# EfficientMoE/MoE-Infinity

Measured on AMD Instinct MI355X. Metric: decode tokens/s through all MoE layers (expert-offload hot path), Mixtral-8x7B, device_memory_ratio=0.75, higher is better.
Workload: dtype bf16

## Files before the change

moe-infinity_amd/csrc/kernels.hip:

```cpp
#include "kdev.h"

#include <algorithm>

#include <type_traits>

#include <string.h>

namespace moeinf {

template <typename T>
__global__ __launch_bounds__(256) void retile_kernel(const T* __restrict__ src, char* __restrict__ dst, int R, int K) {
  constexpr int EPV = DT<T>::EPV;
  constexpr int EPT = 4 * EPV;
  const int KB = (K + EPT - 1) / EPT;
  const int lane = threadIdx.x & 63;
  const int kb = blockIdx.x * 4 + (threadIdx.x >> 6);
  const int rg = blockIdx.y;
  if (kb >= KB) return;
  const int row = rg * 16 + (lane & 15);
  const int k = kb * EPT + (lane >> 4) * EPV;
  u32x4 v = {0u, 0u, 0u, 0u};
  if (row < R && k < K) v = ld16(src + (size_t)row * K + k);
  *reinterpret_cast<u32x4*>(dst + ((size_t)rg * KB + kb) * 1024 + lane * 16) = v;
}
template <typename T>
__global__ __launch_bounds__(256) void retile_blob_kernel(RetileBlob b) {
  constexpr int EPV = DT<T>::EPV;
  constexpr int EPT = 4 * EPV;
  const int t = blockIdx.z;
  const char* src = reinterpret_cast<const char*>(b.src) + b.src_off[t];
  char* dst = reinterpret_cast<char*>(b.dst) + b.dst_off[t];
  const int R = b.R[t], K = b.K[t];
  if (K == 0) {
    const int64_t i = ((int64_t)blockIdx.y * gridDim.x + blockIdx.x) * 256 + threadIdx.x;
    if (i < R) reinterpret_cast<u32x4*>(dst)[i] = reinterpret_cast<const u32x4*>(src)[i];
    return;
  }
  const int KB = (K + EPT - 1) / EPT;
  const int lane = threadIdx.x & 63;
  const int kb = blockIdx.x * 4 + (threadIdx.x >> 6);
  const int rg = blockIdx.y;
  if (kb >= KB || rg * 16 >= R) return;
  const int row = rg * 16 + (lane & 15);
  const int k = kb * EPT + (lane >> 4) * EPV;
  u32x4 v = {0u, 0u, 0u, 0u};
  if (row < R && k < K) v = ld16(reinterpret_cast<const T*>(src) + (size_t)row * K + k);
  *reinterpret_cast<u32x4*>(dst + ((size_t)rg * KB + kb) * 1024 + lane * 16) = v;
}
hipError_t launch_retile_blob(const RetileBlob& b, int dtype, hipStream_t st) {
  const int ept = dtype == DT_F32 ? 16 : 32;
  unsigned gx = 1, gy = 1;
  for (int t = 0; t < b.n; ++t) {
    if (b.K[t] > 0) { gx = std::max(gx, (unsigned)(((b.K[t] + ept - 1) / ept + 3) / 4)); gy = std::max(gy, (unsigned)((b.R[t] + 15) / 16)); }
  }
  for (int t = 0; t < b.n; ++t)
    if (b.K[t] == 0) {
      const int64_t blocks = ((int64_t)b.R[t] + 255) / 256;
      while ((int64_t)gx * gy < blocks) gy += 1;
    }
  const dim3 grid(gx, gy, b.n);
  if (dtype != DT_F32) hipLaunchKernelGGL(retile_blob_kernel<uint16_t>, grid, dim3(256), 0, st, b);
  else hipLaunchKernelGGL(retile_blob_kernel<float>, grid, dim3(256), 0, st, b);
  return hipGetLastError();
}
template <typename T, bool F8>
__global__ __launch_bounds__(256) void pull_retile_kernel(RetileBlob b, unsigned long long* ts, int first) {
  if (ts && first && blockIdx.x == 0 && threadIdx.x == 0) ts[0] = (unsigned long long)wall_clock64();
  constexpr int EPV = DT<T>::EPV;
  constexpr int EPT = 4 * EPV;
  constexpr int W = F8 ? 2 : 1;
  constexpr int CK = 64 * EPV * W;
  constexpr int LROW = 1024 * W + 16;
  __shared__ __attribute__((aligned(16))) char lds[16 * LROW];
  __shared__ uint16_t lut[F8 ? 256 : 1];
  if (F8) {
    const uint32_t v8 = threadIdx.x, sg = v8 >> 7, ex = (v8 >> 3) & 15, m = v8 & 7;
    float f = (ex == 15 && m == 7) ? __builtin_nanf("") : (ex == 0 ? ldexpf((float)m, -9) : ldexpf(1.0f + (float)m * 0.125f, (int)ex - 7));
    if (sg) f = -f;
    lut[v8 & (F8 ? 255 : 0)] = (uint16_t)(__float_as_uint(f) >> 16);
    __syncthreads();
  }
  auto widen = [&](const u32x4 q, u32x4 (&o)[W]) {
    if constexpr (F8) {
      const uint32_t qq[4] = {q.x, q.y, q.z, q.w};
#pragma unroll
      for (int w = 0; w < 2; ++w) {
        uint32_t r4[4];
#pragma unroll
        for (int h2 = 0; h2 < 4; ++h2) {
          const uint32_t ww = qq[w * 2 + (h2 >> 1)], sh = (h2 & 1) * 16;
          r4[h2] = (uint32_t)lut[(ww >> sh) & 255] | ((uint32_t)lut[(ww >> (sh + 8)) & 255] << 16);
        }
        o[w] = u32x4{r4[0], r4[1], r4[2], r4[3]};
      }
    } else {
      o[0] = q;
    }
  };
  const int lane = threadIdx.x & 63, wave = threadIdx.x >> 6;
  int nunit[4], kcs[4], total = 0;
#pragma unroll
  for (int t = 0; t < 4; ++t) {
    kcs[t] = (t < b.n && b.K[t] > 0) ? (b.K[t] + CK - 1) / CK : 1;
    nunit[t] = t < b.n ? (b.K[t] > 0 ? ((b.R[t] + 15) / 16) * kcs[t] : (b.R[t] + 1024 * W - 1) / (1024 * W)) : 0;
    total += nunit[t];
  }
  u32x4 raw[4];
  uint32_t okmask = 0;
  constexpr int SRC_EPL = F8 ? 16 : EPV;
  auto decode = [&](int i, int& t, int& rg, int& kc) {
    t = 0;
    while (t < 3 && i >= nunit[t]) { i -= nunit[t]; ++t; }
    rg = i / kcs[t]; kc = i - rg * kcs[t];
  };
  auto load = [&](int i) {
    int t, rg, kc;
    decode(i, t, rg, kc);
    const char* src = reinterpret_cast<const char*>(b.src) + b.src_off[t];
    constexpr int SRC_ES = F8 ? 1 : (int)sizeof(T);
    okmask = 0;
#pragma unroll
    for (int j = 0; j < 4; ++j) {
      size_t elem;
      bool ok;
      if (b.K[t] > 0) {
        const int row = rg * 16 + wave * 4 + j, k = kc * CK + lane * SRC_EPL;
        ok = row < b.R[t] && k < b.K[t];
        elem = (size_t)min(row, b.R[t] - 1) * b.K[t] + min(k, b.K[t] - SRC_EPL);
      } else {
        const int piece = (rg * 1024 + (wave * 4 + j) * 64 + lane) * W;
        ok = piece < b.R[t];
        elem = (size_t)min(piece, b.R[t] - W) * EPV;
      }
      raw[j] = __builtin_nontemporal_load(reinterpret_cast<const u32x4*>(src + elem * SRC_ES));
      okmask |= (ok ? 1u : 0u) << j;
    }
  };
  int i = blockIdx.x;
  if (i < total) load(i);
  for (; i < total; i += gridDim.x) {
    int t, rg, kc;
    decode(i, t, rg, kc);
#pragma unroll
    for (int j = 0; j < 4; ++j) {
      u32x4 o[W];
      widen(raw[j], o);
#pragma unroll
      for (int w = 0; w < W; ++w) {
        if (!((okmask >> j) & 1u)) o[w] = u32x4{0u, 0u, 0u, 0u};
        *reinterpret_cast<u32x4*>(lds + (wave * 4 + j) * LROW + (lane * W + w) * 16) = o[w];
      }
    }
    __syncthreads();
// ... 348 lines not shown
}
__global__ __launch_bounds__(IDX_THREADS) void index_scatter_kernel(IndexArgs a, const int32_t* __restrict__ chunk_base) {
  const int npairs = a.T * a.K, E = a.E;
  const int p = blockIdx.x * IDX_THREADS + threadIdx.x;
  if (p < npairs) {
    const int rk = a.pair_slot[p];
    if (rk >= 0) {
      const int slot = chunk_base[(size_t)blockIdx.x * E + IDX_AT(a, p)] + rk;
      a.pair_slot[p] = slot;
      a.slot_token[slot] = p / a.K;
      a.slot_pair[slot] = p;
    }
  }
  if (a.shared) {
    const int base = a.offsets[E];
    for (int t = p; t < a.T; t += gridDim.x * IDX_THREADS) {
      a.slot_token[base + t] = t;
      a.slot_pair[base + t] = -1;
    }
  }
}
hipError_t launch_dispatch_index_wide(const IndexArgs& a, int32_t* chunk_scratch, hipStream_t st) {
  const int nchunks = (a.T * a.K + IDX_THREADS - 1) / IDX_THREADS;
  hipLaunchKernelGGL(index_count_kernel, dim3(nchunks), dim3(IDX_THREADS), 0, st, a, chunk_scratch);
  hipLaunchKernelGGL(index_scan_kernel, dim3(1), dim3(IDX_THREADS), 0, st, a, chunk_scratch, nchunks);
  hipLaunchKernelGGL(index_scatter_kernel, dim3(nchunks), dim3(IDX_THREADS), 0, st, a, chunk_scratch);
  return hipGetLastError();
}

hipError_t launch_dispatch_index(const IndexArgs& a, hipStream_t st) {
  hipLaunchKernelGGL(dispatch_index_kernel, dim3(1), dim3(IDX_THREADS), 0, st, a);
  return hipGetLastError();
}

__global__ __launch_bounds__(IDX_THREADS) void route_index_kernel(RouteArgs r, IndexArgs a, EpFuse pk) {
  __shared__ int wave_cnt[IDX_WAVES * IDX_MAXE];
  __shared__ int running[IDX_MAXE];
  __shared__ int offs[IDX_MAXE + 1];
  __shared__ int scan_tmp[IDX_MAXE];
  for (int t = threadIdx.x >> 6; t < r.T; t += IDX_WAVES) route_token(r, t, threadIdx.x & 63);
  __threadfence_block();
  __syncthreads();
  if (a.T * a.K <= 64 && !(a.capacity > 0 && a.T > a.rows)) {
    if (threadIdx.x < 64) index_small(a, running, offs);
  } else {
    index_body(a, wave_cnt, running, offs, scan_tmp);
  }
  if (pk.on) {
    __threadfence_block();
    __syncthreads();
    ep_pack_block_dt(pk, a.T * a.K, scan_tmp);
  }
}

template <typename T, int NW, int U>
__global__ __launch_bounds__(NW * 64) void route_shared2_kernel(RouteArgs r, IndexArgs a, FfnStage s, EpFuse pk) {
  __shared__ int running[IDX_MAXE];
  __shared__ int offs[IDX_MAXE + 1];
  __shared__ float red[NW][1][256];
  if (blockIdx.x == 0) {
    for (int t = threadIdx.x >> 6; t < r.T; t += NW) route_token(r, t, threadIdx.x & 63);
    __threadfence_block();
    __syncthreads();
    if (threadIdx.x < 64) index_small(a, running, offs);
    if (pk.on) {
      __syncthreads();
      ep_pack_block_dt(pk, a.T * a.K, reinterpret_cast<int*>(&red[0][0][0]));
    }
  } else {
    const char* W = reinterpret_cast<const char*>(s.wptr[s.E]);
    ffn_rows_item<T, 1, NW, U, 1>(s, (int)blockIdx.x - 1, W, true, r.T, 0, red);
  }
}
static EpFuse no_pack() {
  EpFuse f;
  memset(&f, 0, sizeof f);
  return f;
}
hipError_t launch_route_shared2(const RouteArgs& r, const IndexArgs& a, const FfnStage& s, hipStream_t st, const EpFuse* pack) {
  static const int nw = env_int("MOEINF_SH2_NW", 8), u = env_int("MOEINF_SH2_U", 4);
  const dim3 grid(1 + (s.R_sh + 15) / 16);
  const EpFuse pk = pack ? *pack : no_pack();
#define RS2(NWV, UU) hipLaunchKernelGGL((route_shared2_kernel<uint16_t, NWV, UU>), grid, dim3(NWV * 64), 0, st, r, a, s, pk)
  if (s.dtype == DT_F16) hipLaunchKernelGGL((route_shared2_kernel<half_t, 8, 4>), grid, dim3(512), 0, st, r, a, s, pk);
  else if (nw == 16) { if (u == 8) RS2(16, 8); else RS2(16, 4); }
  else if (nw == 4) { if (u == 8) RS2(4, 8); else RS2(4, 4); }
  else { if (u == 8) RS2(8, 8); else RS2(8, 4); }
#undef RS2
  return hipGetLastError();
}

template <typename T, int NMAT, int NW, int U>
__global__ __launch_bounds__(NW * 64) __attribute__((amdgpu_num_sgpr(80))) void ffn1_selfroute_kernel(RouteArgs r, IndexArgs a, FfnStage s, FfnStage sh2, int n_rg, int n_sh2) {
  using A = typename act_of<T>::type;
  __shared__ float red[NW][NMAT][256];
  __shared__ unsigned long long sh_w;
  __shared__ int sh_rank_ok;
  static_assert(sizeof(float) * NW * NMAT * 256 >= sizeof(int) * (2 * IDX_MAXE + 1), "index scratch aliases the reduction buffer");
  const int lane = threadIdx.x & 63;
  const int K = r.K, E = r.E;
  int b = (int)blockIdx.x - 1;
  if (n_sh2 < 0) {
    n_sh2 = -n_sh2;
    if (b >= 0) { const int n_routed = (int)gridDim.x - 1 - n_sh2; b = b < n_routed ? b + n_sh2 : b - n_routed; }
  }
  if (b >= 0 && b < n_sh2) {
    const char* Wsh = reinterpret_cast<const char*>(sh2.wptr[sh2.E]);
    ffn_rows_item<A, 1, NW, U, 1>(sh2, b, Wsh, true, 1, 0, reinterpret_cast<float (*)[1][256]>(&red[0][0][0]));
    return;
  }
  b -= n_sh2;
  if (b < 0) {
    if (threadIdx.x < 64) {
      int* scratch = reinterpret_cast<int*>(&red[0][0][0]);
      Routed o;
      route_core(r, 0, lane, o);
      int my_sel, rank;
      float my_w;
      route_store(r, 0, lane, o, &my_sel, &my_w, &rank);
      if (lane < K && s.dec_w) {
        s.dec_w[rank] = my_sel >= 0 ? s.wptr[my_sel] : 0ull;
        s.dec_cw[rank] = my_w;
      }
      __threadfence_block();
      index_small(a, scratch, scratch + IDX_MAXE);
    }
    return;
  }
  const int u = b / n_rg, rg = b - u * n_rg;
  if (threadIdx.x < 64) {
    uint64_t wp = 0;
    if (lane < E) wp = s.wptr[lane];
    uint64_t chosen = route_set_lean(r.logits, E, K, lane, r.kind == 2  ? r.x_dtype : DT_F32);
    for (int i = 0; i < u; ++i) chosen &= chosen - 1;
    const int e = chosen ? (int)__builtin_ctzll(chosen) : -1;
    uint64_t wsel = 0;
    if (e >= 0) {
      const uint32_t lo = (uint32_t)__builtin_amdgcn_readlane((int)(uint32_t)wp, e);
      const uint32_t hi = (uint32_t)__builtin_amdgcn_readlane((int)(uint32_t)(wp >> 32), e);
      wsel = ((uint64_t)hi << 32) | lo;
    }
    if (lane == 0) { sh_w = wsel; sh_rank_ok = e >= 0; }
  }
  __syncthreads();
  if (!sh_rank_ok) return;
  const char* W = reinterpret_cast<const char*>(sh_w);
  if (W == nullptr) {
    if (threadIdx.x == 0 && rg == 0) atomicExch(s.miss_flag, 1);
    return;
  }
  ffn_rows_item<A, NMAT, NW, U, 1, false, false, T>(s, rg, W, false, 1, u, red, 0);
}

static thread_local hipEvent_t t_timer_start = nullptr, t_timer_stop = nullptr;
void arm_kernel_timer(hipEvent_t start, hipEvent_t stop) { t_timer_start = start; t_timer_stop = stop; }
bool take_kernel_timer(hipEvent_t* start, hipEvent_t* stop) {
  if (!t_timer_stop) return false;
  *start = t_timer_start; *stop = t_timer_stop;
  t_timer_start = t_timer_stop = nullptr;
  return true;
}
hipError_t launch_ffn1_selfroute(const RouteArgs& r, const IndexArgs& a, const FfnStage& s1, const FfnStage* sh2, hipStream_t st) {
  const int n_rg = (s1.R + 15) / 16;
  const int n_sh2 = sh2 ? (sh2->R_sh + 15) / 16 : 0;
  const dim3 grid(n_sh2 + r.K * n_rg + 1);
  static const int lds_env = env_int("MOEINF_SR_LDS_KB", -1);
  const size_t dyn = (size_t)(lds_env >= 0 ? lds_env : (grid.x > 4 * 256 ? 30 : 0)) * 1024;
  static const int sr_u_env = env_int("MOEINF_SR_U", 0);
  const int sr_u = sr_u_env ? sr_u_env : (grid.x > 4 * 256 ? 4 : 8);
  if (s1.wdtype == DT_F8) {
    if (s1.epi != EPI_GATED_SILU || s1.dtype != DT_BF16) return hipErrorInvalidValue;
    if (sr_u == 8) KL((ffn1_selfroute_kernel<f8w_t, 2, 4, 8>), grid, dim3(256), dyn, st, r, a, s1, sh2 ? *sh2 : s1, n_rg, n_sh2);
    else KL((ffn1_selfroute_kernel<f8w_t, 2, 4, 4>), grid, dim3(256), dyn, st, r, a, s1, sh2 ? *sh2 : s1, n_rg, n_sh2);
    return hipGetLastError();
  }
  if (s1.epi != EPI_GATED_SILU) {
    if (s1.dtype == DT_BF16) KL((ffn1_selfroute_kernel<uint16_t, 1, 16, 4>), grid, dim3(1024), 0, st, r, a, s1, s1, n_rg, 0);
    else if (s1.dtype == DT_F16) KL((ffn1_selfroute_kernel<half_t, 1, 16, 4>), grid, dim3(1024), 0, st, r, a, s1, s1, n_rg, 0);
    else KL((ffn1_selfroute_kernel<float, 1, 16, 4>), grid, dim3(1024), 0, st, r, a, s1, s1, n_rg, 0);
    return hipGetLastError();
  }
  if (s1.dtype == DT_F16) {
    if (sr_u == 8) KL((ffn1_selfroute_kernel<half_t, 2, 4, 8>), grid, dim3(256), dyn, st, r, a, s1, sh2 ? *sh2 : s1, n_rg, n_sh2);
    else KL((ffn1_selfroute_kernel<half_t, 2, 4, 4>), grid, dim3(256), dyn, st, r, a, s1, sh2 ? *sh2 : s1, n_rg, n_sh2);
    return hipGetLastError();
  }
  static const int sr_order = env_int("MOEINF_SR_ORDER", 0);
  const int n_sh2_arg = (sr_order && n_sh2 > 0) ? -n_sh2 : n_sh2;
  if (sr_u == 8) KL((ffn1_selfroute_kernel<uint16_t, 2, 4, 8>), grid, dim3(256), dyn, st, r, a, s1, sh2 ? *sh2 : s1, n_rg, n_sh2_arg);
  else KL((ffn1_selfroute_kernel<uint16_t, 2, 4, 4>), grid, dim3(256), dyn, st, r, a, s1, sh2 ? *sh2 : s1, n_rg, n_sh2_arg);
  return hipGetLastError();
}

constexpr int SR_MAX_T = 8;
template <typename T, int NW, int U>
__global__ __launch_bounds__(NW * 64) __attribute__((amdgpu_num_sgpr(96))) void ffn1_selfroute_multi_kernel(RouteArgs r, IndexArgs a, FfnStage s, FfnStage sh2, int n_rg, int n_sh2) {
  using A = typename act_of<T>::type;
  __shared__ float red[NW][2][256];
  __shared__ int s_in[SR_MAX_T];
  __shared__ unsigned long long s_w;
  __shared__ int s_cnt, s_off;
  static_assert(sizeof(float) * NW * 2 * 256 >= sizeof(int) * (2 * IDX_MAXE + 1), "index scratch aliases the reduction buffer");
  const int lane = threadIdx.x & 63;
  const int Tn = r.T;
  int blk = (int)blockIdx.x - 1;
  if (blk < 0) {
    for (int t = threadIdx.x >> 6; t < Tn; t += NW) route_token(r, t, lane);
    __threadfence_block();
    __syncthreads();
    if (threadIdx.x < 64) {
      int* scratch = reinterpret_cast<int*>(&red[0][0][0]);
      index_small(a, scratch, scratch + IDX_MAXE);
    }
    return;
  }
  if (blk < n_sh2) {
    const char* Wsh = reinterpret_cast<const char*>(sh2.wptr[sh2.E]);
    ffn_rows_item<A, 1, NW, U, 1>(sh2, blk, Wsh, true, Tn, 0, reinterpret_cast<float (*)[1][256]>(&red[0][0][0]));
    return;
  }
  blk -= n_sh2;
  const int u = blk / n_rg, rg = blk - u * n_rg;
  if (threadIdx.x < 64) {
    uint64_t wp = 0;
    if (lane < r.E) wp = s.wptr[lane];
    uint64_t chosen[SR_MAX_T];
    uint64_t present = 0;
#pragma unroll
    for (int t = 0; t < SR_MAX_T; ++t) {
      chosen[t] = 0;
      if (t < Tn) chosen[t] = route_set_lean(r.logits + (size_t)t * r.E, r.E, r.K, lane);
      present |= chosen[t];
    }
    uint64_t m = present;
    for (int i = 0; i < u; ++i) m &= m - 1;
    const int e = m ? (int)__builtin_ctzll(m) : -1;
    int cnt = 0, off = 0;
    if (e >= 0) {
      const uint64_t below = (1ull << e) - 1ull;
#pragma unroll
      for (int t = 0; t < SR_MAX_T; ++t) {
        off += __popcll(chosen[t] & below);
        if ((chosen[t] >> e) & 1ull) {
          if (lane == 0) s_in[cnt] = t;
          ++cnt;
        }
      }
    }
    uint64_t wsel = 0;
    if (e >= 0) {
      const uint32_t lo = (uint32_t)__builtin_amdgcn_readlane((int)(uint32_t)wp, e);
      const uint32_t hi = (uint32_t)__builtin_amdgcn_readlane((int)(uint32_t)(wp >> 32), e);
      wsel = ((uint64_t)hi << 32) | lo;
    }
    if (lane == 0) { s_w = wsel; s_cnt = cnt; s_off = off; }
  }
  __syncthreads();
  const int cnt = s_cnt;
  if (cnt == 0) return;
  const char* W = reinterpret_cast<const char*>(s_w);
  if (W == nullptr) {
    if (threadIdx.x == 0 && rg == 0) atomicExch(s.miss_flag, 1);
    return;
  }
  ffn_rows_item<A, 2, NW, U, 1, false, false, T>(s, rg, W, false, cnt, s_off, red, -1, s_in, nullptr);
}

hipError_t launch_ffn1_selfroute_multi(const RouteArgs& r, const IndexArgs& a, const FfnStage& s1, const FfnStage* sh2, int max_active, hipStream_t st) {
  const int n_rg = (s1.R + 15) / 16;
  const int n_sh2 = sh2 ? (sh2->R_sh + 15) / 16 : 0;
  const dim3 grid(1 + n_sh2 + max_active * n_rg);
  const size_t dyn = grid.x > 4 * 256 ? 30 * 1024 : 0;
#define SRM(TT, UU) hipLaunchKernelGGL((ffn1_selfroute_multi_kernel<TT, 4, UU>), grid, dim3(256), dyn, st, r, a, s1, sh2 ? *sh2 : s1, n_rg, n_sh2)
  if (s1.wdtype == DT_F8) {
    if (s1.dtype != DT_BF16) return hipErrorInvalidValue;
    if (grid.x > 4 * 256) SRM(f8w_t, 4); else SRM(f8w_t, 8);
  }
  else if (s1.dtype == DT_F16) { if (grid.x > 4 * 256) SRM(half_t, 4); else SRM(half_t, 8); }
  else { if (grid.x > 4 * 256) SRM(uint16_t, 4); else SRM(uint16_t, 8); }
#undef SRM
  return hipGetLastError();
}

template <typename T, int NW, int U>
__global__ __launch_bounds__(NW * 64) void ffn2_decode1_kernel(FfnStage s) {
  using A = typename act_of<T>::type;
  __shared__ float red[NW][1][256];
  __shared__ int is_last;
  const int u = blockIdx.y, tid = threadIdx.x;
  const int K = s.comb.K;
  const char* W = reinterpret_cast<const char*>(s.dec_w[u]);
  CombineMeta m;
#pragma unroll
  for (int kk = 0; kk < 8; ++kk) { m.slot[kk] = min(kk, K - 1); m.w[kk] = s.dec_cw[min(kk, K - 1)]; }
  const int r0 = blockIdx.x * 16;
  if (W == nullptr && tid == 0 && blockIdx.x == 0) atomicExch(s.miss_flag, 1);
  ffn_rows_item<A, 1, NW, U, 1, false, false, T>(s, blockIdx.x, W, false, W ? 1 : 0, u, red);
  wait_stores_acked();
  __syncthreads();
  if (tid == 0) is_last = K == 1 ? 1 : (__hip_atomic_fetch_add(&s.tile_done[blockIdx.x], 1, __ATOMIC_RELAXED, __HIP_MEMORY_SCOPE_AGENT) == K - 1);
  __syncthreads();
  if (is_last) {
    if (s.comb.kind == 2 ) {
      if (tid < 4 && r0 + tid * 4 < s.R) {
        const int h0 = r0 + tid * 4;
        float v[4], o[4];
        DT<A>::unpack4(DT<A>::template fetch4<true>(reinterpret_cast<const A*>(s.comb.y) + h0), v);
        const float pr = s.comb.router_prob[0];
#pragma unroll
        for (int j = 0; j < 4; ++j) o[j] = DT<A>::round(pr * v[j]);
        DT<A>::store4(reinterpret_cast<A*>(s.comb.out) + h0, o);
      }
    } else if (tid < 4) {
      combine_apply<A, true>(s.comb, 0, r0 + tid * 4, m);
    }
    if (tid == 0 && K > 1) s.tile_done[blockIdx.x] = 0;
  }
}

template <typename T, int NWE, int U>
__global__ __launch_bounds__(2 * NWE * 64) void ffn2_decode1_pair_kernel(FfnStage s) {
  using A = typename act_of<T>::type;
  constexpr bool F8W = std::is_same<T, f8w_t>::value;
  constexpr int EPT = F8W ? 64 : 32, EPV = F8W ? 16 : 8;
  __shared__ float red[2][NWE][16];
  __shared__ float yv[2][16];
  const int tid = threadIdx.x, lane = tid & 63, wave = tid >> 6;
  const int g = wave / NWE, wl = wave - g * NWE;
  const int n = lane & 15, q = lane >> 4;
  const int rg = blockIdx.x, r0 = rg * 16;
  const char* W = reinterpret_cast<const char*>(s.dec_w[g]);
  const float cw0 = s.dec_cw[0], cw1 = s.dec_cw[1];
  if (W == nullptr) {
    if (tid == 0 && rg == 0) atomicExch(s.miss_flag, 1);
    return;
  }
  const int KB = s.K / EPT;
  const char* a0 = W + s.off_a + (size_t)rg * KB * 1024 + lane * 16;
  const A* xr = reinterpret_cast<const A*>(s.in) + (size_t)g * s.ld_in + q * EPV;
  f32x4 acc = {0.f, 0.f, 0.f, 0.f};
  if constexpr (F8W) {
    for (int kb = wl; kb < KB; kb += U * NWE) {
      u32x4 av[U], xv[U], xw[U];
#pragma unroll
      for (int i = 0; i < U; ++i) {
        if (kb + i * NWE < KB) {
          av[i] = ld16_nt_global(a0 + (size_t)(kb + i * NWE) * 1024);
          xv[i] = ld16(xr + (size_t)(kb + i * NWE) * EPT);
          xw[i] = ld16(xr + (size_t)(kb + i * NWE) * EPT + 8);
        }
      }
#pragma unroll
      for (int i = 0; i < U; ++i) {
        if (kb + i * NWE < KB) {
          u32x4 lo, hi;
          f8x16_to_bf16(av[i], lo, hi);
          mma16<A>(acc, lo, xv[i]);
          mma16<A>(acc, hi, xw[i]);
        }
      }
    }
  } else
  for (int kb = wl; kb < KB; kb += U * NWE) {
    u32x4 av[U], xv[U];
#pragma unroll
    for (int i = 0; i < U; ++i) {
      if (kb + i * NWE < KB) {
        av[i] = ld16_nt(a0 + (size_t)(kb + i * NWE) * 1024);
        xv[i] = ld16(xr + (size_t)(kb + i * NWE) * EPT);
      }
    }
#pragma unroll
    for (int i = 0; i < U; ++i)
      if (kb + i * NWE < KB) mma16<A>(acc, av[i], xv[i]);
  }
  if (n == 0) {
#pragma unroll
    for (int j = 0; j < 4; ++j) red[g][wl][q * 4 + j] = acc[j];
  }
  __syncthreads();
  if (tid < 32) {
    const int gg = tid >> 4, row = tid & 15;
    float v = 0.f;
#pragma unroll
    for (int w = 0; w < NWE; ++w) v += red[gg][w][row];
    v = DT<A>::round(v);
    yv[gg][row] = v;
    if (r0 + row < s.R) DT<A>::store(reinterpret_cast<A*>(s.out) + (size_t)gg * s.ld_out + r0 + row, v);
  }
  __syncthreads();
  if (tid < 16 && r0 + tid < s.R) {
    float p0 = yv[0][tid] * cw0, p1 = yv[1][tid] * cw1;
    if (s.comb.kind != 1) { p0 = DT<A>::round(p0); p1 = DT<A>::round(p1); }
    float o = DT<A>::round(0.f + p0);
    o = DT<A>::round(o + p1);
    DT<A>::store(reinterpret_cast<A*>(s.comb.out) + r0 + tid, o);
  }
}

hipError_t launch_ffn2_decode1(const FfnStage& s2, hipStream_t st) {
  static const int pair_env = env_int("MOEINF_DEC1_PAIR", 1);
  if (s2.wdtype == DT_F8) {
    if (s2.dtype != DT_BF16 || s2.comb.kind > 1 || (s2.K % 64) != 0) return hipErrorInvalidValue;
    static const int pu = env_int("MOEINF_DEC1_PAIR_U", 4);
    if (pair_env && s2.comb.K == 2 && !(s2.comb.kind == 1 && s2.comb.y_shared)) {
      const dim3 g1((s2.R + 15) / 16);
      if (pu == 8) KL((ffn2_decode1_pair_kernel<f8w_t, 4, 8>), g1, dim3(512), 0, st, s2);
      else KL((ffn2_decode1_pair_kernel<f8w_t, 4, 4>), g1, dim3(512), 0, st, s2);
      return hipGetLastError();
    }
    const dim3 grid((s2.R + 15) / 16, s2.comb.K);
    static const int du = env_int("MOEINF_DEC1_U", 4);
    if ((size_t)s2.K >= 16384) KL((ffn2_decode1_kernel<f8w_t, 8, 4>), grid, dim3(512), 0, st, s2);
    else if (du == 8) KL((ffn2_decode1_kernel<f8w_t, 4, 8>), grid, dim3(256), 0, st, s2);
    else KL((ffn2_decode1_kernel<f8w_t, 4, 4>), grid, dim3(256), 0, st, s2);
    return hipGetLastError();
  }
  if (pair_env && (s2.dtype == DT_BF16 || s2.dtype == DT_F16) && s2.comb.K == 2 && (s2.K % 32) == 0 && !(s2.comb.kind == 1 && s2.comb.y_shared) && s2.comb.kind <= 1) {
    const dim3 g1((s2.R + 15) / 16);
    static const int pu = env_int("MOEINF_DEC1_PAIR_U", 4);
    if (s2.dtype == DT_F16) KL((ffn2_decode1_pair_kernel<half_t, 4, 4>), g1, dim3(512), 0, st, s2);
    else if (pair_env == 8) KL((ffn2_decode1_pair_kernel<uint16_t, 8, 4>), g1, dim3(1024), 0, st, s2);
    else if (pu == 8) KL((ffn2_decode1_pair_kernel<uint16_t, 4, 8>), g1, dim3(512), 0, st, s2);
    else if (pu == 2) KL((ffn2_decode1_pair_kernel<uint16_t, 4, 2>), g1, dim3(512), 0, st, s2);
    else KL((ffn2_decode1_pair_kernel<uint16_t, 4, 4>), g1, dim3(512), 0, st, s2);
    return hipGetLastError();
  }
  const dim3 grid((s2.R + 15) / 16, s2.comb.K);
  if (s2.comb.kind == 2) {
    static const int su = env_int("MOEINF_DEC1_SWITCH_U", 12);
    if (su == 12) {
      if (s2.dtype == DT_BF16) KL((ffn2_decode1_kernel<uint16_t, 16, 12>), grid, dim3(1024), 0, st, s2);
      else if (s2.dtype == DT_F16) KL((ffn2_decode1_kernel<half_t, 16, 12>), grid, dim3(1024), 0, st, s2);
      else KL((ffn2_decode1_kernel<float, 16, 12>), grid, dim3(1024), 0, st, s2);
      return hipGetLastError();
    }
    if (s2.dtype == DT_BF16) KL((ffn2_decode1_kernel<uint16_t, 16, 4>), grid, dim3(1024), 0, st, s2);
    else if (s2.dtype == DT_F16) KL((ffn2_decode1_kernel<half_t, 16, 4>), grid, dim3(1024), 0, st, s2);
    else KL((ffn2_decode1_kernel<float, 16, 4>), grid, dim3(1024), 0, st, s2);
    return hipGetLastError();
  }
  if (s2.dtype == DT_F16) {
    if ((size_t)s2.K * 2 >= 16384) KL((ffn2_decode1_kernel<half_t, 8, 4>), grid, dim3(512), 0, st, s2);
    else KL((ffn2_decode1_kernel<half_t, 4, 4>), grid, dim3(256), 0, st, s2);
    return hipGetLastError();
  }
  const size_t kbytes = (size_t)s2.K * 2;
  static const int du = env_int("MOEINF_DEC1_U", 4);
  if (kbytes >= 16384) KL((ffn2_decode1_kernel<uint16_t, 8, 4>), grid, dim3(512), 0, st, s2);
  else if (du == 8) KL((ffn2_decode1_kernel<uint16_t, 4, 8>), grid, dim3(256), 0, st, s2);
  else if (du == 12) KL((ffn2_decode1_kernel<uint16_t, 4, 12>), grid, dim3(256), 0, st, s2);
  else KL((ffn2_decode1_kernel<uint16_t, 4, 4>), grid, dim3(256), 0, st, s2);
  return hipGetLastError();
}

hipError_t launch_route_index(const RouteArgs& r, const IndexArgs& a, hipStream_t st, const EpFuse* pack) {
  hipLaunchKernelGGL(route_index_kernel, dim3(1), dim3(IDX_THREADS), 0, st, r, a, pack ? *pack : no_pack());
  return hipGetLastError();
}

template <typename MT>
__global__ __launch_bounds__(IDX_THREADS) void mask_index_kernel(const MT* __restrict__ mask, int T, int E, IndexArgs a, const uint8_t* __restrict__ keep) {
  __shared__ int cnt[IDX_MAXE];
  __shared__ int offs[IDX_MAXE + 1];
  const int tid = threadIdx.x, lane = tid & 63, wave = tid >> 6;
  for (int e = wave; e < E; e += IDX_WAVES) {
    int c = 0;
    for (int t0 = 0; t0 < T; t0 += 64) {
      const int t = t0 + lane;
      const bool on = t < T && (!keep || keep[e]) && mask[(size_t)t * E + e] != (MT)0;
      c += __popcll(__ballot(on));
    }
    if (lane == 0) cnt[e] = c;
  }
  __syncthreads();
  if (tid == 0) {
    int acc = 0, na = 0;
    for (int e = 0; e < E; ++e) {
      offs[e] = acc;
      acc += cnt[e];
      if (cnt[e] > 0) a.active[na++] = e;
    }
    offs[E] = acc;
    offs[E + 1] = acc;
    cnt[E] = 0;
    *a.n_active = na;
    if (a.mirror) {
      a.mirror[0] = na;
      for (int i = 0; i < na; ++i) a.mirror[1 + (E + 1) + i] = a.active[i];
      for (int i = na; i <= E; ++i) a.mirror[1 + (E + 1) + i] = -1;
    }
  }
  __syncthreads();
  if (tid <= E) {
    a.counts[tid] = cnt[tid];
    if (a.mirror) a.mirror[1 + tid] = cnt[tid];
  }
  if (tid <= E + 1) a.offsets[tid] = offs[tid];
  for (int e = wave; e < E; e += IDX_WAVES) {
    int base = offs[e];
    for (int t0 = 0; t0 < T; t0 += 64) {
      const int t = t0 + lane;
      const bool on = t < T && (!keep || keep[e]) && mask[(size_t)t * E + e] != (MT)0;
      const uint64_t b = __ballot(on);
      if (on) {
        const int slot = base + __popcll(b & lanes_below(lane));
        if (a.slot_cap <= 0 || slot < a.slot_cap) {
          a.slot_token[slot] = t;
          a.slot_pair[slot] = t * E + e;
        }
      }
      base += __popcll(b);
    }
  }
}
hipError_t launch_mask_index(const void* mask, int mask_elem_bytes, int T, int E, const IndexArgs& a, hipStream_t st, const uint8_t* keep) {
  if (mask_elem_bytes == 1) hipLaunchKernelGGL(mask_index_kernel<uint8_t>, dim3(1), dim3(IDX_THREADS), 0, st, (const uint8_t*)mask, T, E, a, keep);
  else if (mask_elem_bytes == 4) hipLaunchKernelGGL(mask_index_kernel<int32_t>, dim3(1), dim3(IDX_THREADS), 0, st, (const int32_t*)mask, T, E, a, keep);
  else hipLaunchKernelGGL(mask_index_kernel<int64_t>, dim3(1), dim3(IDX_THREADS), 0, st, (const int64_t*)mask, T, E, a, keep);
  return hipGetLastError();
}

__global__ void masked_idx_kernel(const int32_t* __restrict__ idx, const int32_t* __restrict__ valid, int32_t* __restrict__ out, int n) {
  const int i = blockIdx.x * blockDim.x + threadIdx.x;
  if (i < n) out[i] = valid[i] ? idx[i] : -1;
}
hipError_t launch_masked_idx(const int32_t* idx, const int32_t* valid, int32_t* out, int n, hipStream_t st) {
  hipLaunchKernelGGL(masked_idx_kernel, dim3((n + 255) / 256), dim3(256), 0, st, idx, valid, out, n);
  return hipGetLastError();
}

template <typename T>
__global__ __launch_bounds__(256) void combine_kernel(CombineArgs a) {
  const int h0 = (blockIdx.x * 256 + threadIdx.x) * 4;
  if (h0 < a.H) combine_cols<T>(a, blockIdx.y, h0);
}

__global__ void shared_only_index_kernel(IndexArgs a) {
  const int E = a.E, T = a.T;
  for (int e = threadIdx.x; e <= E; e += blockDim.x) { a.counts[e] = (e == E) ? T : 0; a.offsets[e] = 0; }
  if (threadIdx.x == 0) { a.offsets[E + 1] = T; a.active[0] = E; *a.n_active = 1; }
  for (int t = threadIdx.x; t < T; t += blockDim.x) { a.slot_token[t] = t; a.slot_pair[t] = -1; }
}
hipError_t launch_shared_only_index(const IndexArgs& a, hipStream_t st) {
  hipLaunchKernelGGL(shared_only_index_kernel, dim3(1), dim3(256), 0, st, a);
  return hipGetLastError();
}

template <typename T>
__global__ __launch_bounds__(256) void combine_wait_kernel(CombineArgs a, EpWait w) {
  if (threadIdx.x < 64) ep_poll(w.flags, w.n, w.epoch, w.timeout_ticks, w.err);
  __syncthreads();
  const int h0 = (blockIdx.x * 256 + threadIdx.x) * 4;
  if (h0 < a.H) combine_cols<T>(a, blockIdx.y, h0);
}
hipError_t launch_combine(const CombineArgs& a, hipStream_t st, const EpWait* wait) {
  dim3 grid((a.H + 1023) / 1024, a.T);
  if (wait) {
    if (a.dtype == DT_BF16) hipLaunchKernelGGL(combine_wait_kernel<uint16_t>, grid, dim3(256), 0, st, a, *wait);
    else if (a.dtype == DT_F16) hipLaunchKernelGGL(combine_wait_kernel<half_t>, grid, dim3(256), 0, st, a, *wait);
    else hipLaunchKernelGGL(combine_wait_kernel<float>, grid, dim3(256), 0, st, a, *wait);
    return hipGetLastError();
  }
  if (a.dtype == DT_BF16) hipLaunchKernelGGL(combine_kernel<uint16_t>, grid, dim3(256), 0, st, a);
  else if (a.dtype == DT_F16) hipLaunchKernelGGL(combine_kernel<half_t>, grid, dim3(256), 0, st, a);
  else hipLaunchKernelGGL(combine_kernel<float>, grid, dim3(256), 0, st, a);
  return hipGetLastError();
}

__global__ void poke_kernel(PokeArgs a) {
  const int i = threadIdx.x;
  if (i < a.n) a.table[a.idx[i]] = a.val[i];
}
// ... 34 lines not shown
```

Baseline: 280.1.

## Add software-pipelined double-buffered weight streaming for bf16 decode FFN kernels

Adds a decode_stream helper that streams retiled expert weight tiles and activations in batches of U, with two register batches so loads for the next batch are issued while MFMAs consume the current one. New self-routing FFN1 and pair FFN2 decode kernels use this path by default for bf16. The FFN2 default unroll becomes 8, and FFN1 gets a waves_per_eu(4) and SGPR cap hint. The aim is to hide memory latency in the bandwidth-bound decode GEMV. The cost is higher register pressure, which could lower occupancy.

```diff
diff --git a/moe-infinity_amd/csrc/decode_stream.h b/moe-infinity_amd/csrc/decode_stream.h
--- /dev/null
+++ b/moe-infinity_amd/csrc/decode_stream.h
@@ -0,0 +1,135 @@
+#pragma once
+
+#include "kdev.h"
+
+namespace moeinf {
+
+__device__ __forceinline__ u32x4 ld16_global(const void* p) {
+  return *reinterpret_cast<const __attribute__((address_space(1))) u32x4*>(reinterpret_cast<uintptr_t>(p));
+}
+
+template <int NMAT, int U>
+struct DecBatch {
+  u32x4 a[U], b[NMAT == 2 ? U : 1], x[U];
+};
+
+template <int NMAT, int NW, int U>
+__device__ __forceinline__ void dec_load(DecBatch<NMAT, U>& B, const char* a0, const char* a1, const char* xb, const int kb, const int n = U) {
+#pragma unroll
+  for (int i = 0; i < U; ++i) {
+    if (i < n) {
+      B.a[i] = ld16_nt_global(a0 + (size_t)(kb + i * NW) * 1024);
+      if constexpr (NMAT == 2) B.b[i] = ld16_nt_global(a1 + (size_t)(kb + i * NW) * 1024);
+      B.x[i] = ld16_global(xb + (size_t)(kb + i * NW) * 64);
+    }
+  }
+}
+template <int NMAT, int U>
+__device__ __forceinline__ void dec_mma(const DecBatch<NMAT, U>& B, f32x4& acc0, f32x4& acc1, const int n = U) {
+#pragma unroll
+  for (int i = 0; i < U; ++i) {
+    if (i < n) {
+      mma16<uint16_t>(acc0, B.a[i], B.x[i]);
+      if constexpr (NMAT == 2) mma16<uint16_t>(acc1, B.b[i], B.x[i]);
+    }
+  }
+}
+
+template <int NMAT, int NW, int U>
+__device__ __forceinline__ void dec_stream(const char* a0, const char* a1, const char* xb, const int kb0, const int KBfull, const int K,
+                                           f32x4& acc0, f32x4& acc1) {
+  const int kbw = __builtin_amdgcn_readfirstlane(kb0);
+  const int nt = KBfull > kbw ? (KBfull - kbw + NW - 1) / NW : 0;
+  const int nb = nt / U, rem = nt - nb * U;
+  constexpr int STEP = U * NW;
+  int kb = kbw;
+  DecBatch<NMAT, U> A, B;
+  if (nb > 0) {
+    dec_load<NMAT, NW, U>(A, a0, a1, xb, kb);
+    int b = 1;
+    for (; b + 1 < nb; b += 2) {
+      dec_load<NMAT, NW, U>(B, a0, a1, xb, kb + STEP);
+      dec_mma<NMAT, U>(A, acc0, acc1);
+      dec_load<NMAT, NW, U>(A, a0, a1, xb, kb + 2 * STEP);
+      dec_mma<NMAT, U>(B, acc0, acc1);
+      kb += 2 * STEP;
+    }
+    if (b < nb) {
+      dec_load<NMAT, NW, U>(B, a0, a1, xb, kb + STEP);
+      dec_mma<NMAT, U>(A, acc0, acc1);
+      kb += STEP;
+      if (rem) {
+        dec_load<NMAT, NW, U>(A, a0, a1, xb, kb + STEP, rem);
+        dec_mma<NMAT, U>(B, acc0, acc1);
+        dec_mma<NMAT, U>(A, acc0, acc1, rem);
+      } else {
+        dec_mma<NMAT, U>(B, acc0, acc1);
+      }
+    } else if (rem) {
+      dec_load<NMAT, NW, U>(B, a0, a1, xb, kb + STEP, rem);
+      dec_mma<NMAT, U>(A, acc0, acc1);
+      dec_mma<NMAT, U>(B, acc0, acc1, rem);
+    } else {
+      dec_mma<NMAT, U>(A, acc0, acc1);
+    }
+  } else if (rem) {
+    dec_load<NMAT, NW, U>(A, a0, a1, xb, kb, rem);
+    dec_mma<NMAT, U>(A, acc0, acc1, rem);
+  }
+  const int KB = (K + 31) / 32;
+  if (KB != KBfull && kbw == (KBfull % NW)) {
+    const u32x4 z = {0u, 0u, 0u, 0u};
+    const u32x4 w0 = ld16_nt_global(a0 + (size_t)KBfull * 1024);
+    u32x4 w1 = w0;
+    if constexpr (NMAT == 2) w1 = ld16_nt_global(a1 + (size_t)KBfull * 1024);
+    const int kq = ((threadIdx.x & 63) >> 4) * 8;
+    const u32x4 x0 = (KBfull * 32 + kq < K) ? ld16_global(xb + (size_t)KBfull * 64) : z;
+    mma16<uint16_t>(acc0, w0, x0);
+    if constexpr (NMAT == 2) mma16<uint16_t>(acc1, w1, x0);
+  }
+}
+
+template <int NW, int U>
+__device__ __forceinline__ void dec_item_gated(const FfnStage& s, const int bx, const char* W, const int off, float (*red)[2][256]) {
+  using T = uint16_t;
+  const int K = s.K, R = s.R;
+  const int r0 = bx * 16;
+  const int tid = threadIdx.x, lane = tid & 63, wave = tid >> 6;
+  const int KB = (K + 31) / 32, KBfull = K / 32;
+  const char* a0 = W + s.off_a + (size_t)bx * KB * 1024 + lane * 16;
+  const char* a1 = W + s.off_b + (size_t)bx * KB * 1024 + lane * 16;
+  const char* xb = reinterpret_cast<const char*>(s.in) + (lane >> 4) * 16;
+  f32x4 acc0 = {0.f, 0.f, 0.f, 0.f}, acc1 = {0.f, 0.f, 0.f, 0.f};
+  dec_stream<2, NW, U>(a0, a1, xb, wave, KBfull, K, acc0, acc1);
+#pragma unroll
+  for (int j = 0; j < 4; ++j) {
+    red[wave][0][lane * 4 + j] = acc0[j];
+    red[wave][1][lane * 4 + j] = acc1[j];
+  }
+  __syncthreads();
+  for (int i = tid; i < 256; i += NW * 64) {
+    float s0 = 0.f, s1 = 0.f;
+#pragma unroll
+    for (int ww = 0; ww < NW; ++ww) {
+      s0 += red[ww][0][i];
+      s1 += red[ww][1][i];
+    }
+    const int l = i >> 2, j = i & 3;
+    const int orow = r0 + (l >> 4) * 4 + j;
+    if ((l & 15) == 0 && orow < R) {
+      float v = DT<T>::round(s0);
+      const float b = DT<T>::round(s1);
+      if (s.epi == EPI_GATED_SILU) {
+        const float sl = DT<T>::round(v / (1.0f + expf(-v)));
+        v = DT<T>::round(sl * b);
+      } else {
+        const float gl = DT<T>::round(0.5f * v * (1.0f + erff(v * 0.70710678118654752f)));
+        v = DT<T>::round(gl * b);
+      }
+      const int drow = s.out_map ? s.out_map[off] : off;
+      DT<T>::store(reinterpret_cast<T*>(s.out) + (size_t)drow * s.ld_out + orow, v);
+    }
+  }
+}
+
+}
diff --git a/moe-infinity_amd/csrc/kernels.hip b/moe-infinity_amd/csrc/kernels.hip
--- a/moe-infinity_amd/csrc/kernels.hip
+++ b/moe-infinity_amd/csrc/kernels.hip
@@ -1,4 +1,5 @@
 #include "kdev.h"
+#include "decode_stream.h"
 
 #include <algorithm>
 
@@ -653,6 +654,70 @@
   ffn_rows_item<A, NMAT, NW, U, 1, false, false, T>(s, rg, W, false, 1, u, red, 0);
 }
 
+template <int NW, int U>
+__global__ __launch_bounds__(NW * 64) __attribute__((amdgpu_num_sgpr(80), amdgpu_waves_per_eu(4))) void ffn1_selfroute_pipe_kernel(
+    RouteArgs r, IndexArgs a, FfnStage s, FfnStage sh2, int n_rg, int n_sh2) {
+  using A = uint16_t;
+  constexpr int NMAT = 2;
+  __shared__ float red[NW][NMAT][256];
+  __shared__ unsigned long long sh_w;
+  __shared__ int sh_rank_ok;
+  static_assert(sizeof(float) * NW * NMAT * 256 >= sizeof(int) * (2 * IDX_MAXE + 1), "index scratch aliases the reduction buffer");
+  const int lane = threadIdx.x & 63;
+  const int K = r.K, E = r.E;
+  int b = (int)blockIdx.x - 1;
+  if (n_sh2 < 0) {
+    n_sh2 = -n_sh2;
+    if (b >= 0) { const int n_routed = (int)gridDim.x - 1 - n_sh2; b = b < n_routed ? b + n_sh2 : b - n_routed; }
+  }
+  if (b >= 0 && b < n_sh2) {
+    const char* Wsh = reinterpret_cast<const char*>(sh2.wptr[sh2.E]);
+    ffn_rows_item<A, 1, NW, U, 1>(sh2, b, Wsh, true, 1, 0, reinterpret_cast<float (*)[1][256]>(&red[0][0][0]));
+    return;
+  }
+  b -= n_sh2;
+  if (b < 0) {
+    if (threadIdx.x < 64) {
+      int* scratch = reinterpret_cast<int*>(&red[0][0][0]);
+      Routed o;
+      route_core(r, 0, lane, o);
+      int my_sel, rank;
+      float my_w;
+      route_store(r, 0, lane, o, &my_sel, &my_w, &rank);
+      if (lane < K && s.dec_w) {
+        s.dec_w[rank] = my_sel >= 0 ? s.wptr[my_sel] : 0ull;
+        s.dec_cw[rank] = my_w;
+      }
+      __threadfence_block();
+      index_small(a, scratch, scratch + IDX_MAXE);
+    }
+    return;
+  }
+  const int u = b / n_rg, rg = b - u * n_rg;
+  if (threadIdx.x < 64) {
+    uint64_t wp = 0;
+    if (lane < E) wp = s.wptr[lane];
+    uint64_t chosen = route_set_lean(r.logits, E, K, lane, r.kind == 2  ? r.x_dtype : DT_F32);
+    for (int i = 0; i < u; ++i) chosen &= chosen - 1;
+    const int e = chosen ? (int)__builtin_ctzll(chosen) : -1;
+    uint64_t wsel = 0;
+    if (e >= 0) {
+      const uint32_t lo = (uint32_t)__builtin_amdgcn_readlane((int)(uint32_t)wp, e);
+      const uint32_t hi = (uint32_t)__builtin_amdgcn_readlane((int)(uint32_t)(wp >> 32), e);
+      wsel = ((uint64_t)hi << 32) | lo;
+    }
+    if (lane == 0) { sh_w = wsel; sh_rank_ok = e >= 0; }
+  }
+  __syncthreads();
+  if (!sh_rank_ok) return;
+  const char* W = reinterpret_cast<const char*>(sh_w);
+  if (W == nullptr) {
+    if (threadIdx.x == 0 && rg == 0) atomicExch(s.miss_flag, 1);
+    return;
+  }
+  dec_item_gated<NW, U>(s, rg, W, u, red);
+}
+
 static thread_local hipEvent_t t_timer_start = nullptr, t_timer_stop = nullptr;
 void arm_kernel_timer(hipEvent_t start, hipEvent_t stop) { t_timer_start = start; t_timer_stop = stop; }
 bool take_kernel_timer(hipEvent_t* start, hipEvent_t* stop) {
@@ -688,6 +753,12 @@
   }
   static const int sr_order = env_int("MOEINF_SR_ORDER", 0);
   const int n_sh2_arg = (sr_order && n_sh2 > 0) ? -n_sh2 : n_sh2;
+  static const int dec_pipe = env_int("MOEINF_DEC_PIPE", 1);
+  if (dec_pipe && (sr_u == 4 || sr_u == 2)) {
+    if (sr_u == 2) KL((ffn1_selfroute_pipe_kernel<4, 2>), grid, dim3(256), dyn, st, r, a, s1, sh2 ? *sh2 : s1, n_rg, n_sh2_arg);
+    else KL((ffn1_selfroute_pipe_kernel<4, 4>), grid, dim3(256), dyn, st, r, a, s1, sh2 ? *sh2 : s1, n_rg, n_sh2_arg);
+    return hipGetLastError();
+  }
   if (sr_u == 8) KL((ffn1_selfroute_kernel<uint16_t, 2, 4, 8>), grid, dim3(256), dyn, st, r, a, s1, sh2 ? *sh2 : s1, n_rg, n_sh2_arg);
   else KL((ffn1_selfroute_kernel<uint16_t, 2, 4, 4>), grid, dim3(256), dyn, st, r, a, s1, sh2 ? *sh2 : s1, n_rg, n_sh2_arg);
   return hipGetLastError();
@@ -899,6 +970,51 @@
   }
 }
 
+template <int NWE, int U>
+__global__ __launch_bounds__(2 * NWE * 64) void ffn2_decode1_pair_pipe_kernel(FfnStage s) {
+  using A = uint16_t;
+  __shared__ float red[2][NWE][16];
+  __shared__ float yv[2][16];
+  const int tid = threadIdx.x, lane = tid & 63, wave = tid >> 6;
+  const int g = wave / NWE, wl = wave - g * NWE;
+  const int n = lane & 15, q = lane >> 4;
+  const int rg = blockIdx.x, r0 = rg * 16;
+  const char* W = reinterpret_cast<const char*>(s.dec_w[g]);
+  const float cw0 = s.dec_cw[0], cw1 = s.dec_cw[1];
+  if (W == nullptr) {
+    if (tid == 0 && rg == 0) atomicExch(s.miss_flag, 1);
+    return;
+  }
+  const int KB = s.K / 32;
+  const char* a0 = W + s.off_a + (size_t)rg * KB * 1024 + lane * 16;
+  const char* xb = reinterpret_cast<const char*>(s.in) + ((size_t)g * s.ld_in + q * 8) * sizeof(A);
+  f32x4 acc = {0.f, 0.f, 0.f, 0.f}, unused;
+  dec_stream<1, NWE, U>(a0, nullptr, xb, wl, KB, s.K, acc, unused);
+  if (n == 0) {
+#pragma unroll
+    for (int j = 0; j < 4; ++j) red[g][wl][q * 4 + j] = acc[j];
+  }
+  __syncthreads();
+  if (tid < 32) {
+    const int gg = tid >> 4, row = tid & 15;
+    float v = 0.f;
+#pragma unroll
+    for (int w = 0; w < NWE; ++w) v += red[gg][w][row];
+    v = DT<A>::round(v);
+    yv[gg][row] = v;
+    if (r0 + row < s.R) DT<A>::store(reinterpret_cast<A*>(s.out) + (size_t)gg * s.ld_out + r0 + row, v);
+  }
+  __syncthreads();
+  if (tid < 16 && r0 + tid < s.R) {
+    float p0 = yv[0][tid] * cw0, p1 = yv[1][tid] * cw1;
+    if (s.comb.kind != 1) { p0 = DT<A>::round(p0); p1 = DT<A>::round(p1); }
+    float o = DT<A>::round(0.f + p0);
+    o = DT<A>::round(o + p1);
+    DT<A>::store(reinterpret_cast<A*>(s.comb.out) + r0 + tid, o);
+  }
+}
+
+
 hipError_t launch_ffn2_decode1(const FfnStage& s2, hipStream_t st) {
   static const int pair_env = env_int("MOEINF_DEC1_PAIR", 1);
   if (s2.wdtype == DT_F8) {
@@ -919,7 +1035,14 @@
   }
   if (pair_env && (s2.dtype == DT_BF16 || s2.dtype == DT_F16) && s2.comb.K == 2 && (s2.K % 32) == 0 && !(s2.comb.kind == 1 && s2.comb.y_shared) && s2.comb.kind <= 1) {
     const dim3 g1((s2.R + 15) / 16);
-    static const int pu = env_int("MOEINF_DEC1_PAIR_U", 4);
+    static const int pu_env = env_int("MOEINF_DEC1_PAIR_U", 0);
+    static const int dec_pipe = env_int("MOEINF_DEC_PIPE", 1);
+    if (dec_pipe && s2.dtype == DT_BF16 && pair_env != 8 && (pu_env == 0 || pu_env == 4 || pu_env == 8)) {
+      if ((pu_env ? pu_env : 8) == 8) KL((ffn2_decode1_pair_pipe_kernel<4, 8>), g1, dim3(512), 0, st, s2);
+      else KL((ffn2_decode1_pair_pipe_kernel<4, 4>), g1, dim3(512), 0, st, s2);
+      return hipGetLastError();
+    }
+    const int pu = pu_env ? pu_env : 4;
     if (s2.dtype == DT_F16) KL((ffn2_decode1_pair_kernel<half_t, 4, 4>), g1, dim3(512), 0, st, s2);
     else if (pair_env == 8) KL((ffn2_decode1_pair_kernel<uint16_t, 8, 4>), g1, dim3(1024), 0, st, s2);
     else if (pu == 8) KL((ffn2_decode1_pair_kernel<uint16_t, 4, 8>), g1, dim3(512), 0, st, s2);
```

Result: no change. 282.8, median of 6 (+1.0%).
